# Lacadame/DiffSci

Hardware: AMD Instinct MI355X
Metric: samples/sec (50-step Karras Heun), PUNetG 64ch 128x128 (higher is better)
Workload: dtype f32 (3x3 convs: fp16 hi+lo split, 3 fp16 MFMA products, fp32 accumulate); 1 GPU; PUNetG 64-base-ch, 1x128x128 fields, batch 64 per GPU, 50-step Heun deterministic sampler (99 network evaluations); global_batch=64, parallelism=dp1 (batch shards, all-gather of samples), world_size=1, backend=none (one process), hipgraph=True

## Files before the change

diffsci_amd/csrc/ds_conv3p.hip:

```cpp
#include "ds_conv3h_args.h"

#include <atomic>
#include <cstdlib>
#include <type_traits>

namespace ds_conv3 {
namespace {

constexpr int P_WOFF = 2 * XBUF_VEC16 * 16;
constexpr int P_WSLOTS = 4;
constexpr int P_OUTOFF = P_WOFF + P_WSLOTS * WSLAB_VEC * 16;
constexpr int P_BSOFF = P_OUTOFF + 4 * 16384;
constexpr int P_BS_FLOATS = 132;
constexpr int P_LDS = P_BSOFF + 2 * P_BS_FLOATS * 4;
static_assert(P_LDS <= 160 * 1024, "one workgroup per CU");

#ifdef DS_STAMP
#define PSTAMP_SLOTS 64
#define PSTAMP(slot) do { if (a.stamps && (wv == 0 || wv == 4) && lane == 0 && (slot) < PSTAMP_SLOTS) a.stamps[((size_t)blockIdx.x * 2 + (wv >> 2)) * PSTAMP_SLOTS + (slot)] = __builtin_amdgcn_s_memtime(); } while (0)
#else
#define PSTAMP(slot) do {} while (0)
#endif
#ifdef DS_STAMP
#define PSTAMP_FINE(k) do { if (it == 1 && last_of_item) PSTAMP(48 + (k)); } while (0)
#else
#define PSTAMP_FINE(k) do {} while (0)
#endif

#define DS_VMCNT_CASE(n) case n: asm volatile("s_waitcnt vmcnt(" #n ")" ::: "memory"); break;
__device__ __forceinline__ void bar_counted(int young) {
  const int y = __builtin_amdgcn_readfirstlane(young);
  switch (y < 63 ? y : 63) {
    DS_VMCNT_CASE(0) DS_VMCNT_CASE(1) DS_VMCNT_CASE(2) DS_VMCNT_CASE(3) DS_VMCNT_CASE(4) DS_VMCNT_CASE(5) DS_VMCNT_CASE(6) DS_VMCNT_CASE(7)
    DS_VMCNT_CASE(8) DS_VMCNT_CASE(9) DS_VMCNT_CASE(10) DS_VMCNT_CASE(11) DS_VMCNT_CASE(12) DS_VMCNT_CASE(13) DS_VMCNT_CASE(14) DS_VMCNT_CASE(15)
    DS_VMCNT_CASE(16) DS_VMCNT_CASE(17) DS_VMCNT_CASE(18) DS_VMCNT_CASE(19) DS_VMCNT_CASE(20) DS_VMCNT_CASE(21) DS_VMCNT_CASE(22) DS_VMCNT_CASE(23)
    DS_VMCNT_CASE(24) DS_VMCNT_CASE(25) DS_VMCNT_CASE(26) DS_VMCNT_CASE(27) DS_VMCNT_CASE(28) DS_VMCNT_CASE(29) DS_VMCNT_CASE(30) DS_VMCNT_CASE(31)
    DS_VMCNT_CASE(32) DS_VMCNT_CASE(33) DS_VMCNT_CASE(34) DS_VMCNT_CASE(35) DS_VMCNT_CASE(36) DS_VMCNT_CASE(37) DS_VMCNT_CASE(38) DS_VMCNT_CASE(39)
    DS_VMCNT_CASE(40) DS_VMCNT_CASE(41) DS_VMCNT_CASE(42) DS_VMCNT_CASE(43) DS_VMCNT_CASE(44) DS_VMCNT_CASE(45) DS_VMCNT_CASE(46) DS_VMCNT_CASE(47)
    DS_VMCNT_CASE(48) DS_VMCNT_CASE(49) DS_VMCNT_CASE(50) DS_VMCNT_CASE(51) DS_VMCNT_CASE(52) DS_VMCNT_CASE(53) DS_VMCNT_CASE(54) DS_VMCNT_CASE(55)
    DS_VMCNT_CASE(56) DS_VMCNT_CASE(57) DS_VMCNT_CASE(58) DS_VMCNT_CASE(59) DS_VMCNT_CASE(60) DS_VMCNT_CASE(61) DS_VMCNT_CASE(62)
    default: asm volatile("s_waitcnt vmcnt(63)" ::: "memory"); break;
  }
  asm volatile("s_waitcnt lgkmcnt(0)\n\ts_barrier" ::: "memory");
}
#undef DS_VMCNT_CASE

struct Item { int cot, b, y0, x0, tile; };
#define DS_LPI 8

constexpr int XI = 3;
constexpr int BK = 4;
struct Packed { u32x4 h[XI], l[XI]; };
struct ResRegs { f32x4 r1[BK], r2[BK]; };
struct Frag { f16x8 a[2][4], b[2][4]; };

__device__ __forceinline__ void lds_dma16(const void* gsrc, unsigned lane_bytes, unsigned lds) {
  asm volatile("s_mov_b32 m0, %0\n\ts_nop 0\n\tglobal_load_lds_dwordx4 %1, %2" : : "s"(lds), "v"(lane_bytes), "s"(gsrc) : "memory", "m0");
}
__device__ __forceinline__ unsigned lds_address(const void* p) {
  return (unsigned)(unsigned long long)(const __attribute__((address_space(3))) void*)p;
}
__device__ __forceinline__ unsigned const_u32(const void* p, size_t i) {
  typedef const __attribute__((address_space(4))) unsigned* cptr;
  return ((cptr)p)[i];
}

template <bool PRE, bool CIRC, int NRES, bool VEC = false, bool IMG = false>
__global__ __launch_bounds__(512, 2) void k_conv3p(const Conv3hArgs a) {
  static_assert(!IMG || (!PRE && !CIRC && !VEC), "image input: plain zero-padded form");
  constexpr int PW = Geo<false>::PW, NPOS = Geo<false>::NPOS;
  constexpr int HS = NPOS + HPAD16, PS = 2 * NPOS + HPAD16, XBV = XBUF_VEC16;
  extern __shared__ __attribute__((aligned(16))) unsigned char smem[];
  u32x4* Xs = reinterpret_cast<u32x4*>(smem);
  u32x4* Ws = reinterpret_cast<u32x4*>(smem + P_WOFF);
  float* OUT = reinterpret_cast<float*>(smem + P_OUTOFF);
  float* BS = reinterpret_cast<float*>(smem + P_BSOFF);
  const int tid = threadIdx.x, lane = tid & 63;
  const int wv = __builtin_amdgcn_readfirstlane(tid >> 6);
  const bool consumer = wv < 4;
  const int rw = wv & 3;
  const int ptid = tid - 256;
  const int pw = wv - 4;

  const unsigned ntiles = (unsigned)(a.tiles_x * a.tiles_y);
  const unsigned total = (unsigned)a.n_cot * ntiles * (unsigned)a.B;
  const unsigned Q = gridDim.x >> 3, xcd = blockIdx.x & 7u, q = blockIdx.x >> 3;
  const unsigned per = total >> 3, rem = total & 7u;
  const unsigned first = xcd * per + (xcd < rem ? xcd : rem), cnt = per + (xcd < rem ? 1u : 0u);
  const int n_items = q < cnt ? (int)((cnt - q + Q - 1) / Q) : 0;
  if (n_items == 0) return;
  auto div40 = [](unsigned n, unsigned long long magic) __attribute__((always_inline)) { return (unsigned)(((unsigned long long)n * magic) >> 40); };
  auto item_of = [&](int k) __attribute__((always_inline)) {
    const unsigned logical = first + q + Q * (unsigned)k;
    Item it;
    const unsigned rest = div40(logical, a.ncot_magic40);
    it.cot = (int)(logical - rest * (unsigned)a.n_cot);
    const unsigned bb = div40(rest, a.ntiles_magic40);
    it.tile = (int)(rest - bb * ntiles);
    it.b = (int)bb;
    const int ty = a.tiles_x == 1 ? it.tile : (int)__umulhi((unsigned)it.tile, a.tiles_x_magic);
    const int tx = it.tile - ty * a.tiles_x;
    it.y0 = 8 * ty; it.x0 = 32 * tx;
    return it;
  };
  const int n_chunks = a.n_chunks, n_steps = 3 * n_chunks;
  const int HW = a.H * a.W;

  f32x4 acc[4][4];
  const int i16 = lane & 15, h16 = (lane >> 4) & 1, g16 = lane >> 4;
  const bool tapB = lane >= 32;
  const int wlane = h16 * COT + i16;
  int xlane[4];
#pragma unroll
  for (int n = 0; n < 4; ++n) xlane[n] = h16 * HS + (2 * rw + (n >> 1)) * PW + 16 * (n & 1) + i16;
  auto load_pair = [&](Frag& f, int slotA, int kyA, int kxA, int xbA, int slotB, int kyB, int kxB, int xbB) __attribute__((always_inline)) {
    const int wofs = (tapB ? slotB * WSLAB_VEC + kxB * 2 * COT : slotA * WSLAB_VEC + kxA * 2 * COT) + wlane;
    const int xofs = tapB ? xbB * XBV + kyB * PW + kxB : xbA * XBV + kyA * PW + kxA;
#pragma unroll
    for (int p = 0; p < 2; ++p) {
#pragma unroll
      for (int m = 0; m < 4; ++m) f.a[p][m] = *reinterpret_cast<const f16x8*>(&Ws[wofs + p * 6 * COT + 16 * m]);
#pragma unroll
      for (int n = 0; n < 4; ++n) f.b[p][n] = *reinterpret_cast<const f16x8*>(&Xs[xofs + p * PS + xlane[n]]);
    }
  };
  auto mma_pair = [&](const Frag& f) __attribute__((always_inline)) {
    constexpr int PA[3] = {1, 0, 0};
    constexpr int PB[3] = {0, 1, 0};
#pragma unroll
    for (int t = 0; t < 3; ++t)
#pragma unroll
      for (int m = 0; m < 4; ++m)
#pragma unroll
        for (int n = 0; n < 4; ++n)
          acc[m][n] = __builtin_amdgcn_mfma_f32_16x16x32_f16(f.a[PA[t]][m], f.b[PB[t]][n], acc[m][n], 0, 0, 0);
  };
  auto reads_between = [&]() __attribute__((always_inline)) {
    __builtin_amdgcn_sched_group_barrier(0x008, 16, 0);
#pragma unroll
    for (int i = 0; i < 16; ++i) {
      __builtin_amdgcn_sched_group_barrier(0x008, 1, 0);
      __builtin_amdgcn_sched_group_barrier(0x100, 1, 0);
    }
    __builtin_amdgcn_sched_group_barrier(0x008, 16, 0);
  };
  auto park_tile = [&](int par) __attribute__((always_inline)) {
    const float* bs = BS + par * P_BS_FLOATS;
    float* tile = OUT + rw * 4096;
    const float unscale = bs[128];
    float bsv[4][4];
#pragma unroll
    for (int m = 0; m < 4; ++m)
#pragma unroll
      for (int e = 0; e < 4; ++e) {
        const int co = 16 * m + 4 * g16 + e;
        bsv[m][e] = bs[co] + bs[64 + co];
      }
    __builtin_amdgcn_sched_barrier(0);
#pragma unroll
    for (int m = 0; m < 4; ++m)
#pragma unroll
      for (int e = 0; e < 4; ++e) {
        const int co = 16 * m + 4 * g16 + e;
#pragma unroll
        for (int n = 0; n < 4; ++n) {
          tile[(co * 2 + (n >> 1)) * 32 + 16 * (n & 1) + i16] = __builtin_fmaf(acc[m][n][e], unscale, bsv[m][e]);
          acc[m][n][e] = 0.f;
        }
      }
  };

  const int tail_h = (rw >> 1) & 1;
  auto item_h = [&](int i) __attribute__((always_inline)) { (void)pw; return i == 0 ? 0 : (i == 1 ? 1 : tail_h); };
  int xlds[XI], xrow[XI], xcol[XI];
  const bool live_tail = NT + (ptid & (NT / 2 - 1)) < NPOS;
  auto live = [&](int i) __attribute__((always_inline)) { return i < XI - 1 || live_tail; };
#pragma unroll
  for (int i = 0; i < XI; ++i) {
    const int pos = i < 2 ? (ptid & 255) : NT + (ptid & (NT / 2 - 1));
    xrow[i] = pos / PW;
    xcol[i] = pos - xrow[i] * PW;
    xlds[i] = item_h(i) * HS + pos;
  }
  int vr[XI], vx[XI], vch[XI], vlds[XI], vrow[XI];
  const bool halo_live = lane < 20;
  if constexpr (VEC) {
#pragma unroll
    for (int i = 0; i < XI; ++i) {
      vr[i] = 0; vx[i] = 0; vch[i] = 0; vlds[i] = 0; vrow[i] = 0;
      if (i < XI - 1 || pw < 2) {
        const int u = i * 256 + (ptid & 255);
        const int q = u & 3, G = u >> 5;
        const int h = G >= 10 ? 1 : 0, Gp = G - 10 * h;
        int r, g;
        if (Gp < 8) { r = 4 * (Gp >> 2) + ((u >> 3) & 3); g = 2 * (Gp & 3) + ((u >> 2) & 1); }
        else { r = 8 + ((u >> 3) & 1); g = 4 * (Gp - 8) + 2 * ((u >> 4) & 1) + ((u >> 2) & 1); }
        vr[i] = r; vx[i] = 4 * g;
        vch[i] = (8 * h + 2 * q) * HW;
        vlds[i] = 16 * (h * HS + r * PW + 1 + 4 * g) + 4 * q;
        vrow[i] = 8 * h + 2 * q;
      } else {
        const int e = halo_live ? lane : 19, h = pw - 2;
        vr[i] = e >> 1; vx[i] = (e & 1) ? PW - 2 : -1;
        vch[i] = 8 * h * HW;
        vlds[i] = 16 * (h * HS + vr[i] * PW + vx[i] + 1);
        vrow[i] = 8 * h;
      }
    }
  }
  auto pad_vec = [&](int c) __attribute__((always_inline)) { return c < HPAD16 ? NPOS + c : PS + NPOS + (c - HPAD16); };
  constexpr int NINST = (XBV + 63) / 64;
  const int Wp = a.W + 2, Hp = a.H + 2;
  unsigned dbase[6] = {};
  if constexpr (IMG) {
#pragma unroll
    for (int i = 0; i < 6; ++i) {
      const int k = pw + 4 * i;
      const int L = (k < NINST - 1 ? 64 * k : XBV - 64) + lane;
      const int piece = L >= PS ? 1 : 0, Lp = L - piece * PS;
      const int hh = Lp >= HS ? 1 : 0;
      int pos = Lp - hh * HS;
      pos = pos < NPOS ? pos : NPOS - 1;
      const int r = pos / PW, col = pos - r * PW;
      dbase[i] = 16u * (unsigned)(((2 * piece + hh) * Hp + r) * Wp + col);
    }
  }
  int i_k = 0, i_chunk = 0, i_b = 0;
  unsigned i_off = 0;
  auto xdma = [&](int buf) __attribute__((always_inline)) {
    const bool valid = i_k < n_items;
    if (valid && i_chunk == 0) { const Item it = item_of(i_k); i_off = 16u * (unsigned)(it.y0 * Wp + it.x0); i_b = it.b; }
    const u32x4* src = reinterpret_cast<const u32x4*>(a.in) + ((size_t)i_b * n_chunks + i_chunk) * 4 * (size_t)(Hp * Wp);
    u32x4* dst = Xs + buf * XBV;
    int n = 0;
#pragma unroll
    for (int i = 0; i < 6; ++i) {
      const int k = pw + 4 * i;
      if (k < NINST) { lds_dma16(src, dbase[i] + i_off, lds_address(dst + (k < NINST - 1 ? 64 * k : XBV - 64))); ++n; }
    }
    if (valid && ++i_chunk == n_chunks) { i_chunk = 0; ++i_k; }
    return n;
  };
  int f_k = 0, f_chunk = 0, f_b = 0;
  int xoff[XI] = {};
  unsigned f_xvalid = 0;
  float f_in_scale = 1.f;
  auto plan_fetch = [&](const Item& it) __attribute__((always_inline)) {
    f_xvalid = 0;
    if constexpr (VEC) {
#pragma unroll
      for (int i = 0; i < XI; ++i) {
        const bool halo = i == XI - 1 && pw >= 2;
        int gy = it.y0 + vr[i] - 1 + a.oy, gx = it.x0 + vx[i];
        if (CIRC) {
          gy = gy < 0 ? gy + a.H : (gy >= a.H ? gy - a.H : gy);
          gx = gx < 0 ? gx + a.W : (gx >= a.W ? gx - a.W : gx);
          gy = gy >= a.H ? a.H - 1 : gy;
        }
        const bool ok = (!halo || halo_live) && gy >= 0 && gy < a.H && gx >= 0 && gx < a.W;
        xoff[i] = ok ? gy * a.W + gx : 0;
        if (ok) f_xvalid |= 1u << i;
      }
      f_b = it.b;
      if constexpr (!PRE) f_in_scale = ds_epi::act_scale_of(a.in_amax ? const_u32(a.in_amax, it.b) : 0u, a.wshift).in_scale;
      return;
    }
#pragma unroll
    for (int i = 0; i < XI; ++i) {
      int gy = it.y0 + xrow[i] - 1 + a.oy, gx = it.x0 + xcol[i] - 1 + a.ox;
      if (CIRC) {
        gy = gy < 0 ? gy + a.H : (gy >= a.H ? gy - a.H : gy);
        gx = gx < 0 ? gx + a.W : (gx >= a.W ? gx - a.W : gx);
        gy = gy >= a.H ? a.H - 1 : gy;
        gx = gx >= a.W ? a.W - 1 : gx;
      }
      const bool ok = live(i) && gy >= 0 && gy < a.H && gx >= 0 && gx < a.W;
      xoff[i] = ok ? gy * a.W + gx : 0;
      if (ok) f_xvalid |= 1u << i;
    }
    f_b = it.b;
    if constexpr (!PRE) f_in_scale = ds_epi::act_scale_of(a.in_amax ? const_u32(a.in_amax, it.b) : 0u, a.wshift).in_scale;
  };
  const float* f_src = a.in;
  auto fetch_begin = [&](unsigned& tag, int& trow, float& tscale) __attribute__((always_inline)) {
    const bool valid = f_k < n_items;
    if (valid && f_chunk == 0) plan_fetch(item_of(f_k));
    tag = valid ? (0x80000000u | f_xvalid) : 0u;
    trow = (f_b * n_chunks + f_chunk) * KC;
    tscale = f_in_scale;
    f_src = a.in + ((size_t)f_b * a.Cin + (size_t)f_chunk * KC) * HW;
    if (valid && ++f_chunk == n_chunks) { f_chunk = 0; ++f_k; }
  };
  auto fetch_item = [&](auto halo_tag, float (&xr)[XI][8], int i) __attribute__((always_inline)) {
    constexpr bool HALO = decltype(halo_tag)::value;
    if constexpr (VEC) {
      const float* p0 = f_src + vch[i] + xoff[i];
      if (HALO && i == XI - 1) {
#pragma unroll
        for (int k = 0; k < 8; ++k) xr[i][k] = p0[(size_t)k * HW];
      } else {
        const f32x4 t0 = *reinterpret_cast<const f32x4*>(p0);
        const f32x4 t1 = *reinterpret_cast<const f32x4*>(p0 + HW);
#pragma unroll
        for (int k = 0; k < 4; ++k) { xr[i][k] = t0[k]; xr[i][4 + k] = t1[k]; }
      }
    } else {
      const float* p0 = f_src + xoff[i] + (size_t)(8 * item_h(i)) * HW;
#pragma unroll
      for (int k = 0; k < 8; ++k) xr[i][k] = p0[(size_t)k * HW];
    }
  };
  auto fetch_count = [&](auto halo_tag) __attribute__((always_inline)) {
    constexpr bool HALO = decltype(halo_tag)::value;
    return VEC ? (PRE ? 1 : 0) + (HALO ? 2 * (XI - 1) + 8 : 2 * XI) : DS_LPI * XI;
  };
  auto rows_fetch = [&](f32x4& prow, int trow) __attribute__((always_inline)) {
    if constexpr (VEC && PRE) prow = reinterpret_cast<const f32x4*>(a.prenorm)[trow + (lane & 15)];
  };
  auto rows_park = [&](const f32x4& prow, int buf) __attribute__((always_inline)) {
    if constexpr (VEC && PRE) {
      if (pw == 0 && lane < 16) Xs[buf * XBV + pad_vec(lane)] = __builtin_bit_cast(u32x4, prow);
    }
  };
  auto fetch = [&](auto halo_tag, float (&xr)[XI][8], f32x4& prow, unsigned& tag, int& trow, float& tscale) __attribute__((always_inline)) {
    fetch_begin(tag, trow, tscale);
    rows_fetch(prow, trow);
#pragma unroll
    for (int i = 0; i < XI; ++i) fetch_item(halo_tag, xr, i);
    return fetch_count(halo_tag);
  };
  auto activate_item = [&](auto halo_tag, float (&xr)[XI][8], unsigned tag, int trow, float tscale, Packed& pk, int i, int buf) __attribute__((always_inline)) {
    constexpr bool HALO = decltype(halo_tag)::value;
    if constexpr (VEC) {
      if (!(HALO && i == XI - 1)) {
        if constexpr (PRE) {
          const u32x4* rows = Xs + buf * XBV;
          const f32x4 p0 = __builtin_bit_cast(f32x4, rows[pad_vec(vrow[i])]);
          const f32x4 p1 = __builtin_bit_cast(f32x4, rows[pad_vec(vrow[i] + 1)]);
          const float inv = p0[3] == 0.f ? 1.0f : p0[3];
#pragma unroll
          for (int k = 0; k < 4; ++k) {
            xr[i][k] = ds_h3::fast_silu_scaled((xr[i][k] - p0[0]) * p0[1] + p0[2], inv);
            xr[i][4 + k] = ds_h3::fast_silu_scaled((xr[i][4 + k] - p1[0]) * p1[1] + p1[2], inv);
          }
        }
        const bool item_ok = (tag >> i) & 1u;
#pragma unroll
        for (int k = 0; k < 4; ++k) {
          float v0 = item_ok ? xr[i][k] : 0.f;
          float v1 = item_ok ? xr[i][4 + k] : 0.f;
          if constexpr (!PRE) { v0 *= tscale; v1 *= tscale; }
          unsigned ph, pl;
          split2(v0, v1, ph, pl);
          pk.h[i][k] = ph; pk.l[i][k] = pl;
        }
        return;
      }
    }
    if constexpr (PRE) {
      typedef const __attribute__((address_space(4))) f32x4* cptr;
      cptr pp = (cptr)(reinterpret_cast<const f32x4*>(a.prenorm)) + trow;
      const int h = VEC ? pw - 2 : item_h(i);
      f32x4 p[8];
#pragma unroll
      for (int k = 0; k < 8; ++k) p[k] = pp[8 * h + k];
      const float inv = p[0][3] == 0.f ? 1.0f : p[0][3];
#pragma unroll
      for (int k = 0; k < 8; ++k) xr[i][k] = ds_h3::fast_silu_scaled((xr[i][k] - p[k][0]) * p[k][1] + p[k][2], inv);
    }
    const bool item_ok = (tag >> i) & 1u;
#pragma unroll
    for (int k = 0; k < 4; ++k) {
      float v0 = item_ok ? xr[i][2 * k] : 0.f;
      float v1 = item_ok ? xr[i][2 * k + 1] : 0.f;
      if constexpr (!PRE) { v0 *= tscale; v1 *= tscale; }
      unsigned ph, pl;
      split2(v0, v1, ph, pl);
      pk.h[i][k] = ph; pk.l[i][k] = pl;
    }
  };
  auto activate = [&](auto halo_tag, float (&xr)[XI][8], unsigned tag, int trow, float tscale, Packed& pk, int buf) __attribute__((always_inline)) {
#pragma unroll
    for (int i = 0; i < XI; ++i) activate_item(halo_tag, xr, tag, trow, tscale, pk, i, buf);
  };
  auto activate_first_slots = [&](auto halo_tag, float (&xr)[XI][8], unsigned tag, int trow, float tscale, Packed& pk, int buf) __attribute__((always_inline)) {
#pragma unroll
    for (int i = 0; i < XI - 1; ++i) activate_item(halo_tag, xr, tag, trow, tscale, pk, i, buf);
  };
  auto fetch_beside_last_slot = [&](auto halo_tag, float (&xn)[XI][8], f32x4& prown, unsigned& tagn, int& trown, float& tscn,
                                    float (&xo)[XI][8], unsigned tago, int trowo, float tsco, Packed& pk, int bufo) __attribute__((always_inline)) {
    fetch_begin(tagn, trown, tscn);
    rows_fetch(prown, trown);
#pragma unroll
    for (int i = 0; i < XI - 1; ++i) fetch_item(halo_tag, xn, i);
    __builtin_amdgcn_sched_barrier(0);
    activate_item(halo_tag, xo, tago, trowo, tsco, pk, XI - 1, bufo);
    __builtin_amdgcn_sched_barrier(0);
    fetch_item(halo_tag, xn, XI - 1);
    return fetch_count(halo_tag);
  };
  auto store_x = [&](auto halo_tag, const Packed& pk, unsigned tag, int buf) __attribute__((always_inline)) {
    constexpr bool HALO = decltype(halo_tag)::value;
    if (!(tag >> 31)) return;
    if constexpr (VEC) {
      unsigned char* xbytes = smem + (size_t)buf * XBV * 16;
#pragma unroll
      for (int i = 0; i < XI; ++i) {
        if (HALO && i == XI - 1) {
          if (halo_live) {
            *reinterpret_cast<u32x4*>(xbytes + vlds[i]) = pk.h[i];
            *reinterpret_cast<u32x4*>(xbytes + vlds[i] + PS * 16) = pk.l[i];
          }
        } else {
#pragma unroll
          for (int k = 0; k < 4; ++k) {
            *reinterpret_cast<unsigned*>(xbytes + vlds[i] + 16 * k) = pk.h[i][k];
            *reinterpret_cast<unsigned*>(xbytes + vlds[i] + 16 * k + PS * 16) = pk.l[i][k];
          }
        }
      }
      return;
    }
    u32x4* xb = Xs + buf * XBV;
#pragma unroll
    for (int i = 0; i < XI; ++i) {
      if (live(i)) {
        xb[xlds[i]] = pk.h[i];
        xb[PS + xlds[i]] = pk.l[i];
      }
    }
  };
  int w_k = 0, w_step = 0, w_cot = 0;
  constexpr bool cdma = !IMG;
  auto wdma = [&](int slot, int widx) __attribute__((always_inline)) {
    const bool valid = w_k < n_items;
    if (valid && w_step == 0) w_cot = item_of(w_k).cot;
    const u32x4* src = a.wp + ((size_t)w_cot * n_steps + w_step) * WSLAB_VEC;
    u32x4* dst = Ws + slot * WSLAB_VEC;
#pragma unroll
    for (int i = 0; i < 3; ++i) {
      const int k = widx + 4 * i;
      if (k < 12) lds_dma16(src + 64 * k, 16u * (unsigned)lane, lds_address(dst + 64 * k));
    }
    if (valid && ++w_step == n_steps) { w_step = 0; ++w_k; }
    return 0;
  };
  auto bs_fetch = [&](const Item& it, float& vb, float& vs) __attribute__((always_inline)) {
    const int co = it.cot * COT + (ptid & 63);
    vb = a.bias ? a.bias[co] : 0.f;
    vs = a.shift ? a.shift[(size_t)it.b * a.shift_stride + co] : 0.f;
  };
  auto unscale_of = [&](const Item& it) __attribute__((always_inline)) {
    if constexpr (PRE) {
      const float inv = __builtin_bit_cast(float, const_u32(a.prenorm, (size_t)it.b * n_chunks * KC * 4 + 3));
      return ds_epi::unscale_from_inv(inv == 0.f ? 1.0f : inv, a.wshift);
    } else {
      return ds_epi::act_scale_of(a.in_amax ? const_u32(a.in_amax, it.b) : 0u, a.wshift).unscale;
    }
  };
  auto bs_commit = [&](float vb, float vs, float unscale, int par) __attribute__((always_inline)) {
    if (ptid < 128) BS[par * P_BS_FLOATS + ptid] = ptid < 64 ? vb : vs;
    else if (ptid == 128) BS[par * P_BS_FLOATS + 128] = unscale;
  };

  int s_b = 0, s_cot = 0, s_tile = 0;
  size_t s_idx = 0;
  const size_t s_step = 4 * (size_t)HW;
  float s_amax = 0.f;
  const int p4 = 4 * (lane & 7);
  const bool stats = a.tile_stats != nullptr, want_amax = a.out_amax != nullptr;
  constexpr int nres = BK * NRES;
  auto plan_store = [&](const Item& it) __attribute__((always_inline)) {
    s_b = it.b; s_cot = it.cot; s_tile = it.tile;
    const int gy = it.y0 + 2 * rw + ((lane >> 3) & 1), gx = it.x0 + p4;
    const size_t ch = (size_t)it.b * a.Cout + it.cot * COT + (lane >> 4);
    s_idx = ch * HW + (size_t)gy * a.W + gx;
    s_amax = 0.f;
  };
  auto res_prefetch = [&](ResRegs& R, int half) __attribute__((always_inline)) {
#pragma unroll
    for (int k = 0; k < BK; ++k) {
      const int j = half * BK + k;
      if constexpr (NRES >= 1) R.r1[k] = *reinterpret_cast<const f32x4*>(a.res1 + s_idx + (size_t)j * s_step);
      if constexpr (NRES >= 2) R.r2[k] = *reinterpret_cast<const f32x4*>(a.res2 + s_idx + (size_t)j * s_step);
    }
    return nres;
  };
  auto store_batch = [&](const ResRegs& R, int half) __attribute__((always_inline)) {
    float* tile = OUT + rw * 4096;
    f32x4 v[BK];
#pragma unroll
    for (int k = 0; k < BK; ++k) {
      const int seg = (half * BK + k) * 8 + (lane >> 3);
      v[k] = *reinterpret_cast<const f32x4*>(&tile[seg * 32 + p4]);
    }
    if constexpr (NRES >= 1) {
#pragma unroll
      for (int k = 0; k < BK; ++k) v[k] = v[k] + R.r1[k];
    }
    if constexpr (NRES >= 2) {
#pragma unroll
      for (int k = 0; k < BK; ++k) v[k] = v[k] + R.r2[k];
    }
#pragma unroll
    for (int k = 0; k < BK; ++k) *reinterpret_cast<f32x4*>(a.out + s_idx + (size_t)(half * BK + k) * s_step) = v[k];
    if (want_amax) {
#pragma unroll
      for (int k = 0; k < BK; ++k) s_amax = fmaxf(s_amax, ds_epi::abs_max4(v[k]));
    }
    if (stats) {
      f32x4 o[BK];
#pragma unroll
      for (int k = 0; k < BK; ++k) {
        const float K = ds_epi::row16_first(v[k].x);
        const f32x4 d = v[k] - K;
        const float sv = ds_epi::row16_sum((d.x + d.y) + (d.z + d.w));
        const float qv = ds_epi::row16_sum((d.x * d.x + d.y * d.y) + (d.z * d.z + d.w * d.w));
        o[k] = f32x4{K, sv, qv, 64.f};
      }
      if ((lane & 15) == 0) {
#pragma unroll
        for (int k = 0; k < BK; ++k) *reinterpret_cast<f32x4*>(&tile[4 * (4 * (half * BK + k) + (lane >> 4))]) = o[k];
      }
    }
    return BK;
  };
  auto commit_amax_asm = [&]() __attribute__((always_inline)) {
    float m = s_amax;
#pragma unroll
    for (int o = 32; o > 0; o >>= 1) m = fmaxf(m, __shfl_xor(m, o, 64));
    if (lane == 0) atomicMax(a.out_amax + s_b, __builtin_bit_cast(unsigned, m));
  };
  auto store_stats = [&]() __attribute__((always_inline)) {
    const float* tiles = OUT;
    f32x4 pw[4];
#pragma unroll
    for (int w = 0; w < 4; ++w) pw[w] = *reinterpret_cast<const f32x4*>(&tiles[w * 4096 + 4 * lane]);
    const float K = pw[0][0];
    float S = 0.f, Qs = 0.f, n = 0.f;
#pragma unroll
    for (int w = 0; w < 4; ++w) {
      const float dk = pw[w][3] > 0.f ? pw[w][0] - K : 0.f;
      S += pw[w][1] + pw[w][3] * dk;
      Qs += pw[w][2] + 2.f * dk * pw[w][1] + pw[w][3] * dk * dk;
      n += pw[w][3];
    }
    *reinterpret_cast<f32x4*>(a.tile_stats + (((size_t)s_b * a.Cout + s_cot * COT + lane) * ntiles + s_tile) * 4) = f32x4{K, S, Qs, n};
  };

  float xrA[XI][8], xrB[XI][8];
  unsigned tagA = 0, tagB = 0, tagP = 0;
  int trowA = 0, trowB = 0;
  float tscA = 1.f, tscB = 1.f;
  Packed pk;
  f32x4 prowA = {0.f, 0.f, 0.f, 0.f}, prowB = {0.f, 0.f, 0.f, 0.f};
  ResRegs RA, RB;
  float bsb = 0.f, bss = 0.f;
  Frag F0, F1;

  auto run = [&](auto role_tag) __attribute__((always_inline)) {
    constexpr int ROLE = decltype(role_tag)::value;
    constexpr bool CONS = ROLE == 0;
    const std::integral_constant<bool, ROLE == 2> halo{};
    int young = 0, prev = 0, nx = 0;
    constexpr int ndma = 3;
    auto barrier = [&]() __attribute__((always_inline)) {
      if constexpr (CONS) bar_counted(cdma ? 3 : 0);
      else {
        if constexpr (IMG) bar_counted(prev + nx + (cdma ? 0 : ndma) + young);
        else bar_counted(cdma ? 63 : prev + ndma + young);
        prev = young; young = 0; nx = 0;
      }
    };
    int stamp = 1;
    (void)stamp;
    auto chunk_pair = [&](auto base_tag, Frag& Fa, Frag& Fb, bool head, bool second, bool last_of_item, int it) __attribute__((always_inline)) {
      constexpr int B = decltype(base_tag)::value;
      constexpr int E0 = (B + 0) & 3, E1 = (B + 1) & 3, E2 = (B + 2) & 3;
      constexpr int O0 = (B + 3) & 3, O1 = (B + 4) & 3, O2 = (B + 5) & 3;
      constexpr int N0 = (B + 6) & 3;
      constexpr int G[10][8] = {{E0, 0, 0, 0, E0, 0, 1, 0}, {E0, 0, 2, 0, E1, 1, 0, 0}, {E1, 1, 1, 0, E1, 1, 2, 0}, {E2, 2, 0, 0, E2, 2, 1, 0},
                                {E2, 2, 2, 0, O0, 0, 0, 1}, {O0, 0, 1, 1, O0, 0, 2, 1}, {O1, 1, 0, 1, O1, 1, 1, 1}, {O1, 1, 2, 1, O2, 2, 0, 1},
                                {O2, 2, 1, 1, O2, 2, 2, 1}, {N0, 0, 0, 0, N0, 0, 1, 0}};
      auto group = [&](auto k_tag) __attribute__((always_inline)) {
        constexpr int k = decltype(k_tag)::value;
        Frag& cur = (k & 1) ? Fb : Fa;
        Frag& nxt = (k & 1) ? Fa : Fb;
        load_pair(nxt, G[k + 1][0], G[k + 1][1], G[k + 1][2], G[k + 1][3], G[k + 1][4], G[k + 1][5], G[k + 1][6], G[k + 1][7]);
        mma_pair(cur);
        reads_between();
      };
#define DS_GROUP(k) group(std::integral_constant<int, k>{})
      if constexpr (CONS) {
        if (cdma) { wdma((B + 3) & 3, rw); __builtin_amdgcn_sched_barrier(0); }
        if (head) park_tile((it - 1) & 1);
        DS_GROUP(0); DS_GROUP(1);
      } else {
        if constexpr (IMG) nx = xdma(1);
        if (!cdma) wdma((B + 3) & 3, pw);
        __builtin_amdgcn_sched_barrier(0);
        if (head) { plan_store(item_of(it - 1)); young += res_prefetch(RA, 0); }
        if constexpr (!IMG) {
          young += fetch_beside_last_slot(halo, xrB, prowB, tagB, trowB, tscB, xrA, tagA, trowA, tscA, pk, 1);
          tagP = tagA;
        }
      }
      if (stamp < 48) PSTAMP(stamp);
      ++stamp;
      barrier();
      if constexpr (CONS) {
        if (cdma) { wdma((B + 4) & 3, rw); __builtin_amdgcn_sched_barrier(0); }
        DS_GROUP(2);
      } else {
        if (!cdma) wdma((B + 4) & 3, pw);
        __builtin_amdgcn_sched_barrier(0);
        if constexpr (!IMG) {
          store_x(halo, pk, tagP, 1);
          rows_park(prowB, 0);
        }
        if (head) {
          young += store_batch(RA, 0);
          young += res_prefetch(RB, 1);
        }
        if (second) { young += store_batch(RA, 2); young += res_prefetch(RB, 3); }
      }
      if (stamp < 48) PSTAMP(stamp);
      ++stamp;
      barrier();
      if constexpr (CONS) {
        if (cdma) { wdma((B + 5) & 3, rw); __builtin_amdgcn_sched_barrier(0); }
        DS_GROUP(3); DS_GROUP(4);
      } else {
        if (!cdma) wdma((B + 5) & 3, pw);
        __builtin_amdgcn_sched_barrier(0);
        if constexpr (!IMG) activate_first_slots(halo, xrB, tagB, trowB, tscB, pk, 0);
        __builtin_amdgcn_sched_barrier(0);
      }
      if (stamp < 48) PSTAMP(stamp);
      ++stamp;
      barrier();
      if constexpr (CONS) {
        if (cdma) { wdma((B + 6) & 3, rw); __builtin_amdgcn_sched_barrier(0); }
        DS_GROUP(5);
      } else {
        PSTAMP_FINE(0);
        if constexpr (IMG) nx = xdma(0);
        if (!cdma) wdma((B + 6) & 3, pw);
        __builtin_amdgcn_sched_barrier(0);
        PSTAMP_FINE(1);
        if constexpr (!IMG) young += fetch_beside_last_slot(halo, xrA, prowA, tagA, trowA, tscA, xrB, tagB, trowB, tscB, pk, 0);
        __builtin_amdgcn_sched_barrier(0);
        PSTAMP_FINE(2);
        if (last_of_item && it + 1 < n_items) bs_fetch(item_of(it + 1), bsb, bss);
      }
      if (stamp < 48) PSTAMP(stamp);
      ++stamp;
      barrier();
      if constexpr (CONS) {
        if (cdma) { wdma((B + 7) & 3, rw); __builtin_amdgcn_sched_barrier(0); }
        DS_GROUP(6); DS_GROUP(7);
      } else {
        PSTAMP_FINE(4);
        if (!cdma) wdma((B + 7) & 3, pw);
        __builtin_amdgcn_sched_barrier(0);
        PSTAMP_FINE(5);
        if constexpr (!IMG) {
          store_x(halo, pk, tagB, 0);
          rows_park(prowA, 1);
        }
        PSTAMP_FINE(6);
        if (head) { young += store_batch(RB, 1); young += res_prefetch(RA, 2); }
        if (second) { young += store_batch(RB, 3); if (want_amax) commit_amax_asm(); }
      }
      if (stamp < 48) PSTAMP(stamp);
      ++stamp;
      barrier();
      if constexpr (CONS) {
        if (cdma) { wdma((B + 8) & 3, rw); __builtin_amdgcn_sched_barrier(0); }
        DS_GROUP(8);
      } else {
        if (!cdma) wdma((B + 8) & 3, pw);
        __builtin_amdgcn_sched_barrier(0);
        if constexpr (!IMG) activate_first_slots(halo, xrA, tagA, trowA, tscA, pk, 1);
        __builtin_amdgcn_sched_barrier(0);
        if (second && stats && wv == 4) store_stats();
        if (last_of_item && it + 1 < n_items) bs_commit(bsb, bss, unscale_of(item_of(it + 1)), (it + 1) & 1);
      }
      if (stamp < 48) PSTAMP(stamp);
      ++stamp;
      barrier();
#undef DS_GROUP
    };

    {
      const unsigned skew = (blockIdx.x * 11u) & (unsigned)a.pc_skew_mask;
      for (unsigned i = 0; i < skew; ++i) __builtin_amdgcn_s_sleep(8);
    }
    if constexpr (!CONS) {
      if constexpr (IMG) xdma(0);
      if (!cdma) { wdma(0, pw); wdma(1, pw); wdma(2, pw); }
      if constexpr (!IMG) {
        fetch(halo, xrB, prowB, tagB, trowB, tscB);
        fetch(halo, xrA, prowA, tagA, trowA, tscA);
      }
      bs_fetch(item_of(0), bsb, bss);
      if constexpr (VEC && PRE) {
        asm volatile("s_waitcnt vmcnt(0)" ::: "memory");
        rows_park(prowB, 0);
        rows_park(prowA, 1);
        asm volatile("s_waitcnt lgkmcnt(0)\n\ts_barrier" ::: "memory");
      }
      if constexpr (!IMG) {
        activate(halo, xrB, tagB, trowB, tscB, pk, 0);
        store_x(halo, pk, tagB, 0);
        activate_first_slots(halo, xrA, tagA, trowA, tscA, pk, 1);
      }
      bs_commit(bsb, bss, unscale_of(item_of(0)), 0);
      if constexpr (VEC || IMG) asm volatile("s_waitcnt vmcnt(0)" ::: "memory");
      else asm volatile("s_waitcnt vmcnt(20)" ::: "memory");
    } else {
      if (cdma) { wdma(0, rw); wdma(1, rw); wdma(2, rw); }
      if constexpr (VEC && PRE) asm volatile("s_waitcnt lgkmcnt(0)\n\ts_barrier" ::: "memory");
#pragma unroll
      for (int m = 0; m < 4; ++m)
#pragma unroll
        for (int n = 0; n < 4; ++n)
#pragma unroll
          for (int e = 0; e < 4; ++e) acc[m][n][e] = 0.f;
    }
    PSTAMP(0);
    if constexpr (CONS) asm volatile("s_waitcnt vmcnt(0)" ::: "memory");
    asm volatile("s_waitcnt lgkmcnt(0)\n\ts_barrier" ::: "memory");
    young = 0; prev = (VEC || IMG) ? 0 : DS_LPI * XI;
    if constexpr (CONS) load_pair(F0, 0, 0, 0, 0, 0, 0, 1, 0);

    const int ncp = n_chunks >> 1;
    for (int it = 0; it < n_items; ++it) {
      for (int cp = 0; cp < ncp; cp += 2) {
        chunk_pair(std::integral_constant<int, 0>{}, F0, F1, cp == 0 && it > 0, false, false, it);
        chunk_pair(std::integral_constant<int, 6>{}, F1, F0, false, cp == 0 && it > 0, cp + 2 == ncp, it);
      }
    }
    if constexpr (CONS) {
      park_tile((n_items - 1) & 1);
    } else {
      plan_store(item_of(n_items - 1));
      res_prefetch(RA, 0);
    }
    bar_counted(0);
    if constexpr (!CONS) {
      store_batch(RA, 0);
      res_prefetch(RB, 1);
    }
    bar_counted(0);
    if constexpr (!CONS) {
      store_batch(RB, 1);
      res_prefetch(RA, 2);
      store_batch(RA, 2);
      res_prefetch(RB, 3);
      store_batch(RB, 3);
      if (want_amax) commit_amax_asm();
    }
    bar_counted(0);
    if constexpr (!CONS) {
      if (stats && wv == 4) store_stats();
    }
  };
  if (consumer) {
    run(std::integral_constant<int, 0>{});
  } else {
    if (a.pc_prio == 1) __builtin_amdgcn_s_setprio(1);
    else if (a.pc_prio == 2) __builtin_amdgcn_s_setprio(2);
    else if (a.pc_prio == 3) __builtin_amdgcn_s_setprio(3);
    if (VEC && pw >= 2) run(std::integral_constant<int, VEC ? 2 : 1>{});
    else run(std::integral_constant<int, 1>{});
  }
}

template <bool PRE, bool CIRC, int NRES, bool VEC = false, bool IMG = false>
int launch_conv3p_w(const Conv3hArgs& a, int wgs, hipStream_t s) {
  const int rc = ds::ensure_dynamic_lds<&k_conv3p<PRE, CIRC, NRES, VEC, IMG>>(P_LDS, "hipFuncSetAttribute(conv3p)");
  if (rc != DS_OK) return rc;
  hipLaunchKernelGGL((k_conv3p<PRE, CIRC, NRES, VEC, IMG>), dim3((unsigned)wgs), dim3(512), P_LDS, s, a);
  DS_CHECK_LAUNCH("ds_conv2d_h3 (persistent)");
  return DS_OK;
}
bool conv3p_vec() {
  static const bool on = [] { const char* e = getenv("DS_CONV_VEC"); return !(e && atoi(e) == 0); }();
  return on;
}
template <bool PRE, bool CIRC, int NRES>
int launch_conv3p_r(const Conv3hArgs& a, int wgs, hipStream_t s) {
  if (conv3p_vec() && a.ox == 0 && (reinterpret_cast<uintptr_t>(a.in) & 15u) == 0) return launch_conv3p_w<PRE, CIRC, NRES, true>(a, wgs, s);
  return launch_conv3p_w<PRE, CIRC, NRES>(a, wgs, s);
}
void conv3p_fill_args(Conv3hArgs& a) {
  a.ntiles_magic40 = (1ull << 40) / (unsigned long long)(a.tiles_x * a.tiles_y) + 1ull;
  a.ncot_magic40 = (1ull << 40) / (unsigned long long)a.n_cot + 1ull;
  static const int prio = [] { const char* e = getenv("DS_CONV_PC_PRIO"); const int v = e ? atoi(e) : 0; return v < 0 || v > 3 ? 0 : v; }();
  a.pc_prio = prio;
  static const int skew = [] { const char* e = getenv("DS_CONV_PC_SKEW"); const int v = e ? atoi(e) : 0; return v < 0 || v > 31 ? 0 : v; }();
  a.pc_skew_mask = skew;
  if (!a.res1 && a.res2) { a.res1 = a.res2; a.res2 = nullptr; }
}
template <bool PRE, bool CIRC>
int launch_conv3p(Conv3hArgs a, int wgs, hipStream_t s) {
  conv3p_fill_args(a);
  if (!a.res1) return launch_conv3p_r<PRE, CIRC, 0>(a, wgs, s);
  return a.res2 ? launch_conv3p_r<PRE, CIRC, 2>(a, wgs, s) : launch_conv3p_r<PRE, CIRC, 1>(a, wgs, s);
}

int conv3p_mode() {
  static const int v = [] { const char* e = getenv("DS_CONV_PC"); return e ? atoi(e) : 2; }();
  return v;
}
int conv3p_min_items() {
  static const int v = [] { const char* e = getenv("DS_CONV_PC_MIN"); const int n = e ? atoi(e) : 1; return n < 1 ? 1 : n; }();
  return v;
}
int conv3p_cus() {
  static std::atomic<int> cus[64];
  int dev = 0;
  if (hipGetDevice(&dev) != hipSuccess) return 256;
  int c = cus[dev & 63].load(std::memory_order_acquire);
  if (c == 0) {
    hipDeviceProp_t p;
    c = hipGetDeviceProperties(&p, dev) == hipSuccess ? p.multiProcessorCount : 256;
    cus[dev & 63].store(c, std::memory_order_release);
  }
  return c;
}

}

int conv3p_try_launch_img(const Conv3hArgs& a0, hipStream_t s, bool* launched) {
  *launched = false;
  static const bool on = [] { const char* e = getenv("DS_CONV_PC_IMG"); return !(e && atoi(e) == 0); }();
  if (!on || conv3p_mode() == 0) return DS_OK;
  if (a0.H % 8 != 0 || a0.W % 32 != 0 || a0.Cout % COT != 0 || a0.Cin % (4 * KC) != 0 || a0.res1_up) return DS_OK;
  const long long total = (long long)a0.n_cot * a0.tiles_x * a0.tiles_y * a0.B;
  const int wgs = conv3p_cus() / 8 * 8;
  if (wgs <= 0 || total < (long long)wgs * conv3p_min_items() || total >= (1ll << 22)) return DS_OK;
  if ((long long)4 * (a0.H + 2) * (a0.W + 2) * 16 >= (1ll << 31)) return DS_OK;
  Conv3hArgs a = a0;
  conv3p_fill_args(a);
  int rc;
  if (!a.res1) rc = launch_conv3p_w<false, false, 0, false, true>(a, wgs, s);
  else rc = a.res2 ? launch_conv3p_w<false, false, 2, false, true>(a, wgs, s) : launch_conv3p_w<false, false, 1, false, true>(a, wgs, s);
  if (rc == DS_OK) *launched = true;
  return rc;
}

int conv3p_try_launch(const Conv3hArgs& a, hipStream_t s, bool* launched) {
  *launched = false;
  const int mode = conv3p_mode();
  if (mode == 0) return DS_OK;
  if (a.H % 8 != 0 || a.W % 32 != 0 || a.Cout % COT != 0 || a.Cin % (4 * KC) != 0) return DS_OK;
  if (a.Hin != a.H || a.Win != a.W || a.res1_up) return DS_OK;
  const long long total = (long long)a.n_cot * a.tiles_x * a.tiles_y * a.B;
  const int wgs = conv3p_cus() / 8 * 8;
  if (wgs <= 0 || total < (long long)wgs * conv3p_min_items() || total >= (1ll << 22)) return DS_OK;
  if (a.n_cot % 2 == 0 && a.prenorm && mode < 2) return DS_OK;
  if (!a.prenorm && mode < 3) return DS_OK;
  int rc;
  if (a.prenorm) rc = a.circular ? launch_conv3p<true, true>(a, wgs, s) : launch_conv3p<true, false>(a, wgs, s);
  else rc = a.circular ? launch_conv3p<false, true>(a, wgs, s) : launch_conv3p<false, false>(a, wgs, s);
  if (rc == DS_OK) *launched = true;
  return rc;
}

}
```

Measured before the change: 84.11 samples/s.

## Overlap accumulator parking with first MFMA product and swizzle LDS output tile

The consumer waves now write the previous item's accumulators to the LDS output tile interleaved with the first MFMA product of the next item. Each first product seeds acc from zero, so the separate zeroing pass is gone. MFMA operands are swapped so each lane holds four consecutive positions per output channel, allowing vectorized f32x4 LDS stores into an XOR-swizzled layout, and the store path reads the tile with the matching swizzle. A dummy bias-scale commit for parity slot 1 ensures the first item's park reads defined values, in exchange for more complex scheduling and a changed tile layout.

```diff
diff --git a/diffsci_amd/csrc/ds_conv3p.hip b/diffsci_amd/csrc/ds_conv3p.hip
--- a/diffsci_amd/csrc/ds_conv3p.hip
+++ b/diffsci_amd/csrc/ds_conv3p.hip
@@ -124,19 +124,22 @@
       for (int n = 0; n < 4; ++n) f.b[p][n] = *reinterpret_cast<const f16x8*>(&Xs[xofs + p * PS + xlane[n]]);
     }
   };
+  constexpr int PA[3] = {1, 0, 0};
+  constexpr int PB[3] = {0, 1, 0};
+  auto mma_product = [&](const Frag& f, auto t_tag) __attribute__((always_inline)) {
+    constexpr int t = decltype(t_tag)::value;
+#pragma unroll
+    for (int m = 0; m < 4; ++m)
+#pragma unroll
+      for (int n = 0; n < 4; ++n)
+        acc[m][n] = __builtin_amdgcn_mfma_f32_16x16x32_f16(f.b[PB[t]][n], f.a[PA[t]][m], acc[m][n], 0, 0, 0);
+  };
   auto mma_pair = [&](const Frag& f) __attribute__((always_inline)) {
-    constexpr int PA[3] = {1, 0, 0};
-    constexpr int PB[3] = {0, 1, 0};
-#pragma unroll
-    for (int t = 0; t < 3; ++t)
-#pragma unroll
-      for (int m = 0; m < 4; ++m)
-#pragma unroll
-        for (int n = 0; n < 4; ++n)
-          acc[m][n] = __builtin_amdgcn_mfma_f32_16x16x32_f16(f.a[PA[t]][m], f.b[PB[t]][n], acc[m][n], 0, 0, 0);
-  };
-  auto reads_between = [&]() __attribute__((always_inline)) {
-    __builtin_amdgcn_sched_group_barrier(0x008, 16, 0);
+    mma_product(f, std::integral_constant<int, 0>{});
+    mma_product(f, std::integral_constant<int, 1>{});
+    mma_product(f, std::integral_constant<int, 2>{});
+  };
+  auto reads_between_tail = [&]() __attribute__((always_inline)) {
 #pragma unroll
     for (int i = 0; i < 16; ++i) {
       __builtin_amdgcn_sched_group_barrier(0x008, 1, 0);
@@ -144,29 +147,46 @@
     }
     __builtin_amdgcn_sched_group_barrier(0x008, 16, 0);
   };
+  auto reads_between = [&]() __attribute__((always_inline)) {
+    __builtin_amdgcn_sched_group_barrier(0x008, 16, 0);
+    reads_between_tail();
+  };
+  typedef f32x4 __attribute__((address_space(3))) * lds_f32x4;
+  unsigned pq[4];
+#pragma unroll
+  for (int n = 0; n < 4; ++n) pq[n] = lds_address(OUT) + 4u * (unsigned)(rw * 4096 + 64 * i16 + 4 * ((4 * n + g16) ^ i16));
+  auto park_rows = [&](int par, float& unscale, float (&bsv)[4]) __attribute__((always_inline)) {
+    const float* bs = BS + par * P_BS_FLOATS;
+    unscale = bs[128];
+#pragma unroll
+    for (int m = 0; m < 4; ++m) bsv[m] = bs[16 * m + i16] + bs[64 + 16 * m + i16];
+    __builtin_amdgcn_sched_barrier(0);
+  };
+  auto park_block = [&](int m, int n, float unscale, const float (&bsv)[4]) __attribute__((always_inline)) {
+    f32x4 v;
+#pragma unroll
+    for (int e = 0; e < 4; ++e) v[e] = __builtin_fmaf(acc[m][n][e], unscale, bsv[m]);
+    *(lds_f32x4)(size_t)(pq[n] + 4096u * (unsigned)m) = v;
+  };
   auto park_tile = [&](int par) __attribute__((always_inline)) {
-    const float* bs = BS + par * P_BS_FLOATS;
-    float* tile = OUT + rw * 4096;
-    const float unscale = bs[128];
-    float bsv[4][4];
+    float unscale, bsv[4];
+    park_rows(par, unscale, bsv);
 #pragma unroll
     for (int m = 0; m < 4; ++m)
 #pragma unroll
-      for (int e = 0; e < 4; ++e) {
-        const int co = 16 * m + 4 * g16 + e;
-        bsv[m][e] = bs[co] + bs[64 + co];
-      }
-    __builtin_amdgcn_sched_barrier(0);
+      for (int n = 0; n < 4; ++n) park_block(m, n, unscale, bsv);
+  };
+  auto park_under_product = [&](const Frag& f, int par) __attribute__((always_inline)) {
+    float unscale, bsv[4];
+    park_rows(par, unscale, bsv);
+    const f32x4 zero = {0.f, 0.f, 0.f, 0.f};
 #pragma unroll
     for (int m = 0; m < 4; ++m)
 #pragma unroll
-      for (int e = 0; e < 4; ++e) {
-        const int co = 16 * m + 4 * g16 + e;
-#pragma unroll
-        for (int n = 0; n < 4; ++n) {
-          tile[(co * 2 + (n >> 1)) * 32 + 16 * (n & 1) + i16] = __builtin_fmaf(acc[m][n][e], unscale, bsv[m][e]);
-          acc[m][n][e] = 0.f;
-        }
+      for (int n = 0; n < 4; ++n) {
+        park_block(m, n, unscale, bsv);
+        acc[m][n] = __builtin_amdgcn_mfma_f32_16x16x32_f16(f.b[PB[0]][n], f.a[PA[0]][m], zero, 0, 0, 0);
+        __builtin_amdgcn_sched_barrier(0);
       }
   };
 
@@ -491,8 +511,8 @@
     f32x4 v[BK];
 #pragma unroll
     for (int k = 0; k < BK; ++k) {
-      const int seg = (half * BK + k) * 8 + (lane >> 3);
-      v[k] = *reinterpret_cast<const f32x4*>(&tile[seg * 32 + p4]);
+      const int co = (half * BK + k) * 4 + (lane >> 4);
+      v[k] = *reinterpret_cast<const f32x4*>(&tile[co * 64 + 4 * ((lane & 15) ^ (co & 15))]);
     }
     if constexpr (NRES >= 1) {
 #pragma unroll
@@ -574,8 +594,9 @@
     };
     int stamp = 1;
     (void)stamp;
-    auto chunk_pair = [&](auto base_tag, Frag& Fa, Frag& Fb, bool head, bool second, bool last_of_item, int it) __attribute__((always_inline)) {
+    auto chunk_pair = [&](auto base_tag, auto first_tag, Frag& Fa, Frag& Fb, bool head, bool second, bool last_of_item, int it) __attribute__((always_inline)) {
       constexpr int B = decltype(base_tag)::value;
+      constexpr bool FIRST = decltype(first_tag)::value;
       constexpr int E0 = (B + 0) & 3, E1 = (B + 1) & 3, E2 = (B + 2) & 3;
       constexpr int O0 = (B + 3) & 3, O1 = (B + 4) & 3, O2 = (B + 5) & 3;
       constexpr int N0 = (B + 6) & 3;
@@ -590,11 +611,19 @@
         mma_pair(cur);
         reads_between();
       };
+      auto group0_head = [&](int par) __attribute__((always_inline)) {
+        park_under_product(Fa, par);
+        load_pair(Fb, G[1][0], G[1][1], G[1][2], G[1][3], G[1][4], G[1][5], G[1][6], G[1][7]);
+        mma_product(Fa, std::integral_constant<int, 1>{});
+        mma_product(Fa, std::integral_constant<int, 2>{});
+        reads_between_tail();
+      };
 #define DS_GROUP(k) group(std::integral_constant<int, k>{})
       if constexpr (CONS) {
         if (cdma) { wdma((B + 3) & 3, rw); __builtin_amdgcn_sched_barrier(0); }
-        if (head) park_tile((it - 1) & 1);
-        DS_GROUP(0); DS_GROUP(1);
+        if constexpr (FIRST) group0_head((it - 1) & 1);
+        else DS_GROUP(0);
+        DS_GROUP(1);
       } else {
         if constexpr (IMG) nx = xdma(1);
         if (!cdma) wdma((B + 3) & 3, pw);
@@ -716,6 +745,7 @@
         activate_first_slots(halo, xrA, tagA, trowA, tscA, pk, 1);
       }
       bs_commit(bsb, bss, unscale_of(item_of(0)), 0);
+      bs_commit(0.f, 0.f, 0.f, 1);
       if constexpr (VEC || IMG) asm volatile("s_waitcnt vmcnt(0)" ::: "memory");
       else asm volatile("s_waitcnt vmcnt(20)" ::: "memory");
     } else {
@@ -735,10 +765,21 @@
     if constexpr (CONS) load_pair(F0, 0, 0, 0, 0, 0, 0, 1, 0);
 
     const int ncp = n_chunks >> 1;
+    const std::integral_constant<int, 0> b0{};
+    const std::integral_constant<int, 6> b6{};
     for (int it = 0; it < n_items; ++it) {
-      for (int cp = 0; cp < ncp; cp += 2) {
-        chunk_pair(std::integral_constant<int, 0>{}, F0, F1, cp == 0 && it > 0, false, false, it);
-        chunk_pair(std::integral_constant<int, 6>{}, F1, F0, false, cp == 0 && it > 0, cp + 2 == ncp, it);
+      if constexpr (CONS) {
+        chunk_pair(b0, std::true_type{}, F0, F1, false, false, false, it);
+        chunk_pair(b6, std::false_type{}, F1, F0, false, false, false, it);
+        for (int cp = 2; cp < ncp; cp += 2) {
+          chunk_pair(b0, std::false_type{}, F0, F1, false, false, false, it);
+          chunk_pair(b6, std::false_type{}, F1, F0, false, false, false, it);
+        }
+      } else {
+        for (int cp = 0; cp < ncp; cp += 2) {
+          chunk_pair(b0, std::false_type{}, F0, F1, cp == 0 && it > 0, false, false, it);
+          chunk_pair(b6, std::false_type{}, F1, F0, false, cp == 0 && it > 0, cp + 2 == ncp, it);
+        }
       }
     }
     if constexpr (CONS) {
```

New measurement: 84.37 samples/s (median of 3 runs). About the same (+0.3%).
